# TLeconte/vdlm2dec

Measured on AMD Instinct MI355X. Metric: IQ MS/s demodulated (8 ch, 2 MS/s cs16) + CRC-pass frame parity vs ref, higher is better.
Workload: dtype f32

## Files before the change

### vdlm2dec_amd/csrc/vdl2gpu.hip

```cpp
#include "vdl2gpu_kernels.h"
#include "vdl2gpu_blocks.h"

#include <algorithm>
#include <cmath>
#include <cstdio>
#include <cstdlib>
#include <chrono>
#include <cstring>
#include <mutex>
#include <new>
#include <string>
#include <type_traits>
#include <vector>

extern "C" void sincosf(float, float *, float *);

#define HIPCHK(h, expr)                                                                         \
	do {                                                                                    \
		hipError_t e__ = (expr);                                                        \
		if (e__ != hipSuccess) {                                                        \
			(h)->err = std::string(#expr) + ": " + hipGetErrorString(e__);          \
			return VDL2GPU_EHIP;                                                    \
		}                                                                               \
	} while (0)
// ... 982 lines not shown
	HIPCHK(h, hipStreamSynchronize(h->stream));
	return VDL2GPU_OK;
}

extern "C" int vdl2gpu_create(const vdl2gpu_config_t *cfg, vdl2gpu_t **out)
{
	if (!cfg || !out || cfg->struct_size != sizeof(vdl2gpu_config_t))
		return VDL2GPU_EINVAL;
	if (cfg->nbch < 1 || cfg->nbch > VDL2GPU_MAXCH || cfg->nstreams < 1 || !cfg->chan || !cfg->max_push)
		return VDL2GPU_EINVAL;
	if (fmt_bytes(cfg->fmt) == 0 || cfg->sdrinrate < 100000)
		return VDL2GPU_EINVAL;
	const bool offgrid = cfg->sdrinrate % 25000 != 0;
	if (offgrid && (cfg->sdrinrate % 1000 || (cfg->flags & VDL2GPU_F_RTL_QUIRK)))
		return VDL2GPU_EINVAL;
	if ((cfg->flags & VDL2GPU_F_RTL_QUIRK) && cfg->fmt != VDL2GPU_FMT_CU8)
		return VDL2GPU_EINVAL;
	if (cfg->flags & VDL2GPU_F_EXACT_FO) {
		if (cfg->flags & VDL2GPU_F_RTL_QUIRK)
			return VDL2GPU_EINVAL;
		for (size_t i = 0; i < (size_t)cfg->nstreams * cfg->nbch; ++i)
			if (2ll * std::llabs((long long)cfg->chan[i].Fo) >= (long long)cfg->sdrinrate)
				return VDL2GPU_EINVAL;
	}
#ifndef VDL2GPU_TESTHOOKS
	if (cfg->flags & VDL2GPU_F_TEST_NOREGION)
		return VDL2GPU_EINVAL;
#endif
	const unsigned sdrclk = cfg->sdrclk ? cfg->sdrclk : cfg->sdrinrate / 4000;
	if (sdrclk <= 21 || sdrclk > 1000000)
		return VDL2GPU_EINVAL;
	const unsigned lo_len = (unsigned)vdl2gpu_lo_len(cfg->sdrinrate);
	if (offgrid) {
		if ((4ull * sdrclk) % lo_len || k1_win_bytes((sdrclk + 20) / 21) > VDL2_K1_LDS_MAX)
			return VDL2GPU_EINVAL;
	} else if (k1_smem_bytes(lo_len, (sdrclk + 20) / 21) > VDL2_K1_LDS_MAX)
		return VDL2GPU_EINVAL;
	const long long cap = plane_frames(cfg->max_push, sdrclk);
	if (cap == 0 || (unsigned long long)cap * VDL2_CS * sizeof(float2) >= VDL2_PLANES_MAX)
		return VDL2GPU_EINVAL;
	vdl2gpu_t *h = new(std::nothrow) vdl2gpu;
	if (!h)
		return VDL2GPU_ENOMEM;
	h->cfg = *cfg;
	h->S = cfg->nstreams;
	h->C = cfg->nbch;
	h->L = (int)lo_len;
	h->sdrclk = (int)sdrclk;
	h->maxwin = (h->sdrclk + 20) / 21;
	h->k1_glo = offgrid && k1_smem_bytes((uint64_t)h->L, (uint64_t)h->maxwin) > VDL2_K1_LDS_MAX;
	h->sample_bytes = fmt_bytes(cfg->fmt);
	h->rec_cap = cfg->max_bursts ? cfg->max_bursts : 65536u;
	h->chans.assign(cfg->chan, cfg->chan + (size_t)cfg->nstreams * cfg->nbch);
	h->cfg.chan = h->chans.data();
	const int rc = create_impl(h);
	if (rc != VDL2GPU_OK) {
		std::string e = h->err;
		if (getenv("VDL2GPU_VERBOSE"))
			fprintf(stderr, "vdl2gpu_create: %s\n", e.c_str());
		vdl2gpu_destroy(h);
		*out = nullptr;
		return rc;
	}
	*out = h;
	return VDL2GPU_OK;
}

static int get_events(vdl2gpu_t *h, PushTiming &pt)
{
	if (!h->free_ev.empty()) {
		pt = h->free_ev.back();
		h->free_ev.pop_back();
		return VDL2GPU_OK;
	}
	for (auto &e : pt.e)
		NEW_EVENT(h, e, true);
	return VDL2GPU_OK;
}

static int harvest_timing(vdl2gpu_t *h)
{
	for (auto &pt : h->pending) {
		float d[NEV - 1] = {0};
		if (h->stage_dump && pt.staged && h->ev_origin) {
			static const int order[] = {0, 1, 10, 4, 2, 13, 23, 14, 12, 15, 16, 18, 5, 20, 21, 22, 6, 7};
			fprintf(stderr, "vdl2gpu stage dump push %llu:", (unsigned long long)pt.index);
			for (int k : order) {
				float t = -1.0f;
				if (hipEventElapsedTime(&t, h->ev_origin, pt.e[k]) != hipSuccess) {
					(void)hipGetLastError();
					t = -1.0f;
				}
				fprintf(stderr, " e%d=%.1f", k, t * 1e3f);
			}
			fprintf(stderr, "\n");
		}
		for (int i = 0; i + 1 < NEV; ++i) {
			if (!pt.staged)
				break;
			if (i == 3)
				HIPCHK(h, hipEventElapsedTime(&d[i], pt.e[13], pt.e[14]));
			else
				HIPCHK(h, hipEventElapsedTime(&d[i], i == 1 ? pt.e[10] : (i == 4 ? pt.e[12] : pt.e[i]), i == 1 ? pt.e[4] : pt.e[i + 1]));
		}
		if (pt.fast && pt.staged) {
			float a = 0, b = 0, c = 0;
			HIPCHK(h, hipEventElapsedTime(&a, pt.e[0], pt.e[11]));
			HIPCHK(h, hipEventElapsedTime(&b, pt.e[8], pt.e[9]));
			HIPCHK(h, hipEventElapsedTime(&c, pt.e[9], pt.e[1]));
			d[0] = a + b + c;
		}
		if (pt.staged) {
			h->st_k1 += d[0];
			h->st_scan += d[1] + d[4];
			h->st_cluster += d[2];
			h->st_resolve += d[3] + d[5];
			h->st_demod += d[1] + d[2] + d[3] + d[4] + d[5];
			h->st_other += d[6];
			h->st_pushes++;
		}
		if (pt.fast && pt.staged) {
			float f = 0;
			HIPCHK(h, hipEventElapsedTime(&f, pt.e[8], pt.e[9]));
			h->tm.channelise_fast_ms += f;
			h->tm.fast_pushes++;
		}
		h->tm.pushes++;
		h->tm.samples += pt.samples;
		h->free_ev.push_back(pt);
	}
	h->pending.clear();
	return VDL2GPU_OK;
}

static int harvest_ring(vdl2gpu_t *h, int ring, bool blocking);
static int enqueue_back(vdl2gpu_t *h);
static void spill_slab(vdl2gpu_t *h, int slab);

enum { SCAN_PROBE, SCAN_REGION, SCAN_VERIFY };
struct ScanDrain { int slot = -1, mode = 0, skip = 0, pch = 0, nwg = 0; };
static void scan_drain(K2Params &q, const ScanDrain &d)
{
	q.drain_slot = d.slot;
	q.drain_mode = d.mode;
	q.drain_skip = d.skip;
	q.drain_pch = d.pch;
	q.drain_nwg = d.nwg;
}
static ScanDrain launch_scan(int which, const K2Params &k2, dim3 grid, hipStream_t st, int slot, int mode, int skip, unsigned tiles_per_wg)
{
	K2Params q = k2;
	const unsigned item_priv = k2.item_priv;
	grid.x = std::min<unsigned>(grid.x, VDL2_MAXWG);
	if (which != SCAN_VERIFY)
		grid.x = std::max(1u, std::min<unsigned>(grid.x, item_priv / 256u));
	unsigned want = (tiles_per_wg * (which == SCAN_REGION ? 400u : 42u * (K2A_TS / 1024u)) + 128u + 255u) / 256u * 256u;
	q.surv_common_cap = 0;
#ifdef VDL2GPU_TESTHOOKS
	const bool test_items = !g_test_item_verify || which == SCAN_VERIFY;
	if (test_items && g_test_item_grid > 0) {
		grid.x = std::min<unsigned>(grid.x, (unsigned)g_test_item_grid);
		want = 256u;
	}
	if (test_items && g_test_item_common > 0)
		q.surv_common_cap = g_test_item_common;
#endif
	q.surv_nwg = (int)grid.x;
	q.surv_pch = (int)std::max(256u, std::min(want, item_priv / grid.x / 256u * 256u));
	q.surv_slot = slot;
	q.surv_mode = mode;
	q.surv_skip = skip;
	q.drain_slot = -1;
	switch (which) {
	case SCAN_PROBE: hipLaunchKernelGGL(k2a_probe, grid, dim3(K2A_THREADS), 0, st, q); break;
	case SCAN_REGION: hipLaunchKernelGGL(k2a_region, grid, dim3(K2A_THREADS), 0, st, q); break;
	default: hipLaunchKernelGGL(k2a_verify, grid, dim3(K2A_THREADS), 0, st, q); break;
	}
	ScanDrain d;
	d.slot = slot;
	d.mode = mode;
	d.skip = skip;
	d.pch = q.surv_pch;
	d.nwg = q.surv_nwg;
	return d;
}

template <class F> static void with_fmt(int fmt, F &&f)
{
	switch (fmt) {
	case VDL2GPU_FMT_CU8: f(std::integral_constant<int, VDL2GPU_FMT_CU8>{}); break;
	case VDL2GPU_FMT_CS16: f(std::integral_constant<int, VDL2GPU_FMT_CS16>{}); break;
	case VDL2GPU_FMT_CF32: f(std::integral_constant<int, VDL2GPU_FMT_CF32>{}); break;
	case VDL2GPU_FMT_CS8: f(std::integral_constant<int, VDL2GPU_FMT_CS8>{}); break;
	case VDL2GPU_FMT_S16R: f(std::integral_constant<int, VDL2GPU_FMT_S16R>{}); break;
	default: f(std::integral_constant<int, VDL2GPU_FMT_F32R>{}); break;
	}
}

static int push_impl(vdl2gpu_t *h, const void *iq, size_t nsamples, size_t stream_stride_bytes, int memkind, bool wait_copy);

static int push_checked(vdl2gpu_t *h, const void *iq, size_t nsamples, size_t stream_stride_bytes, int memkind, bool wait_copy)
{
	if (h && h->failed) {
		h->err = "an earlier HIP error left the handle unusable: " + h->err;
		return VDL2GPU_EHIP;
	}
	int rc = VDL2GPU_OK;
	const size_t lim = h ? h->split_samples : 0;
	auto passes = [&](const void *q, size_t n) -> int { return push_impl(h, q, n, stream_stride_bytes, memkind, wait_copy); };
	if (!h || !iq || lim == 0 || nsamples <= lim)
		rc = passes(iq, nsamples);
	else {
		if (nsamples > h->cfg.max_push)
			return VDL2GPU_EINVAL;
		const size_t parts = (nsamples + lim - 1) / lim;
		const size_t unit = h->split_unit;
		const size_t part = ((nsamples + parts - 1) / parts + unit - 1) / unit * unit;
		for (size_t off = 0; off < nsamples && rc == VDL2GPU_OK; off += part)
			rc = passes((const char *)iq + off * h->sample_bytes, std::min(part, nsamples - off));
	}
	if (rc == VDL2GPU_EHIP)
		h->failed = true;
	return rc;
}

extern "C" int vdl2gpu_push(vdl2gpu_t *h, const void *iq, size_t nsamples, size_t stream_stride_bytes, int memkind)
{
	if (!h)
		return VDL2GPU_EINVAL;
	HLOCK(h);
	return push_checked(h, iq, nsamples, stream_stride_bytes, memkind, true);
}

extern "C" int vdl2gpu_ring_init(vdl2gpu_t *h, size_t slot_samples, int nslots)
{
	if (!h || slot_samples == 0 || slot_samples > h->cfg.max_push || nslots < 2 || nslots > 64)
		return VDL2GPU_EINVAL;
	HLOCK(h);
	if (h->ring_host) {
		h->err = "vdl2gpu_ring_init: the ring exists already";
		return VDL2GPU_EINVAL;
	}
	HIPCHK(h, hipSetDevice(h->cfg.device));
	h->ring_slot_samples = slot_samples;
	h->ring_slot_bytes = slot_samples * h->sample_bytes * (size_t)h->S;
	HOST_ALLOC(h, h->ring_host, h->ring_slot_bytes * (size_t)nslots, hipHostMallocDefault);
	h->ring_nslots = nslots;
	h->ring_copied.resize((size_t)nslots);
	h->ring_inflight.assign((size_t)nslots, 0);
	for (int i = 0; i < nslots; ++i)
		NEW_EVENT(h, h->ring_copied[(size_t)i]);
	return VDL2GPU_OK;
}

extern "C" void *vdl2gpu_ring_acquire(vdl2gpu_t *h, size_t *stream_stride_bytes)
{
	if (!h)
		return nullptr;
	HLOCK(h);
	if (!h->ring_host || h->ring_acquired)
		return nullptr;
	const size_t slot = (size_t)(h->ring_next % (unsigned long long)h->ring_nslots);
	if (h->ring_inflight[slot]) {
		if (hipSetDevice(h->cfg.device) != hipSuccess || hipEventSynchronize(h->ring_copied[slot]) != hipSuccess) {
			h->err = "vdl2gpu_ring_acquire: waiting for the slot failed";
			return nullptr;
		}
		h->ring_inflight[slot] = 0;
	}
	if (stream_stride_bytes)
		*stream_stride_bytes = h->ring_slot_samples * h->sample_bytes;
	h->ring_acquired = true;
	return (char *)h->ring_host + slot * h->ring_slot_bytes;
}

extern "C" int vdl2gpu_ring_commit(vdl2gpu_t *h, size_t nsamples)
{
	if (!h)
		return VDL2GPU_EINVAL;
	HLOCK(h);
	if (!h->ring_host || !h->ring_acquired || nsamples > h->ring_slot_samples)
		return VDL2GPU_EINVAL;
	const size_t slot = (size_t)(h->ring_next % (unsigned long long)h->ring_nslots);
	h->ring_acquired = false;
	h->ring_next++;
	if (nsamples == 0)
		return VDL2GPU_OK;
	const int rc = push_checked(h, (char *)h->ring_host + slot * h->ring_slot_bytes, nsamples,
				    h->ring_slot_samples * h->sample_bytes, VDL2GPU_MEM_HOST, false);
	if (h->in_stream) {
		if (hipEventRecord(h->ring_copied[slot], h->in_stream) == hipSuccess)
			h->ring_inflight[slot] = 1;
		else if (rc == VDL2GPU_OK) {
			h->err = "hipEventRecord(ring_copied)";
			h->failed = true;
			return VDL2GPU_EHIP;
		}
	}
	return rc;
}


static inline void (*k2d_kernel(const vdl2gpu_t *h))(K2Params)
{
	return h->col_on[COL_SOFT] ? (h->col_on[COL_LEVEL] ? k2d_payload_lev_soft : k2d_payload_soft) : (h->col_on[COL_LEVEL] ? k2d_payload_lev : k2d_payload);
}

static int enqueue_back(vdl2gpu_t *h)
{
	if (!h->back.valid)
		return VDL2GPU_OK;
	h->back.valid = false;
	const K2Params &k2 = h->back.k2;
	const int64_t J = h->back.J;
	const int par = h->back.par, ring = h->back.ring;
	const bool staged = h->back.staged, serial = h->back.serial;
	const unsigned tiles = h->back.tiles;
	const int GS = h->S;
	PushTiming &pt = h->pending[h->back.pt_index];
	const dim3 gch((unsigned)h->C, (unsigned)GS);
	hipStream_t rs = h->stream;
	if (h->back.two_streams)
		HIPCHK(h, hipStreamWaitEvent(rs, h->set[par].f_done, 0));
	if (staged)
		HIPCHK(h, hipEventRecord(pt.e[2], rs));
	if (!serial)
		hipLaunchKernelGGL(k2b_clusters, dim3((unsigned)(h->n_cu * 4 * K2B_GRIDW), (unsigned)((GS * VDL2_CS + 63) / 64)), dim3(K2B_NT), 0, rs, k2);
	HIPCHK(h, hipGetLastError());
	if (staged)
		HIPCHK(h, hipEventRecord(pt.e[3], rs));
	if (staged)
		HIPCHK(h, hipEventRecord(pt.e[13], rs));
	const dim3 vgrid0((tiles / 2 + 1 + K2A_VRUN - 1) / K2A_VRUN, (unsigned)h->C, (unsigned)GS);
	ScanDrain vdrain;
	if (h->k2f_rec)
		HIPCHK(h, hipStreamWaitEvent(rs, h->k2f_done, 0));
	if (staged && h->stage_dump)
		HIPCHK(h, hipEventRecord(pt.e[23], rs));
	hipLaunchKernelGGL(k2c_resolve, gch, dim3(K2_NT), 0, rs, k2);
	HIPCHK(h, hipGetLastError());
	if (staged)
		HIPCHK(h, hipEventRecord(pt.e[14], rs));
	const bool spec = !h->full_scan && !serial && h->S * VDL2_CS <= 512;
	h->ring[ring].spec = spec;
	if (spec)
		HIPCHK(h, hipEventRecord(h->k2c_done, rs));
	hipStream_t ps = h->copy_stream;
	if (spec) {
		HIPCHK(h, hipStreamWaitEvent(ps, h->k2c_done, 0));
		hipLaunchKernelGGL(k2d_kernel(h), dim3((unsigned)h->k2d_grid, (unsigned)(VDL2_CS * GS)), dim3(K2D_NT), 0, ps, k2);
		HIPCHK(h, hipEventRecord(h->pay_done, ps));
	}
	if (staged)
		HIPCHK(h, hipEventRecord(pt.e[12], h->stream));
	if (!serial)
		vdrain = launch_scan(SCAN_VERIFY, k2, vgrid0, h->stream, VDL2_SURV_VERIFY, 1, 0, K2A_VRUN);
	HIPCHK(h, hipGetLastError());
	if (staged && h->stage_dump)
		HIPCHK(h, hipEventRecord(pt.e[15], h->stream));
	hipStream_t ts = (spec && h->back.two_streams && !h->knob.no_tail) ? h->pay_stream : h->stream;
	if (ts != h->stream) {
		HIPCHK(h, hipEventRecord(h->verify_done, h->stream));
		HIPCHK(h, hipStreamWaitEvent(ts, h->verify_done, 0));
	}
	if (h->tail_prev && h->tail_prev != ts && h->set[(par + VDL2_NSET - 1) % VDL2_NSET].k2_rec)
		HIPCHK(h, hipStreamWaitEvent(ts, h->set[(par + VDL2_NSET - 1) % VDL2_NSET].k2_done, 0));
	h->tail_prev = ts;
	if (staged && h->stage_dump)
		HIPCHK(h, hipEventRecord(pt.e[16], ts));
	if (!h->full_scan && !serial) {
		K2Params k2r = k2;
		if (spec && h->repair_rounds >= 2 && ts != ps)
			HIPCHK(h, hipStreamWaitEvent(ts, h->pay_done, 0));
		const dim3 vgrid((tiles / 2 + 1 + K2A_VRUN - 1) / K2A_VRUN, (unsigned)h->C, (unsigned)GS);
		for (int rr = 1; rr <= h->repair_rounds; ++rr) {
			k2r.round = rr;
			k2r.full_round = (rr == h->repair_rounds && h->repair_rounds >= 2) ? 1 : 0;
			k2r.mini_round = k2r.full_round ? 0 : 1;
			if (k2r.full_round) {
				scan_drain(k2r, vdrain);
				hipLaunchKernelGGL(k2r_regions, gch, dim3(K2R_NT), 0, ts, k2r);
				scan_drain(k2r, ScanDrain());
				const unsigned want = tiles;
				unsigned per = (unsigned)h->n_cu;
				per = per > want ? want : per;
				const ScanDrain pdrain = launch_scan(SCAN_PROBE, k2r, dim3(per, (unsigned)h->C, (unsigned)GS), ts, VDL2_SURV_FULL, 0, 0, 4 * ((want + per - 1) / per));
				scan_drain(k2r, pdrain);
				hipLaunchKernelGGL(k2s_sort, gch, dim3(K2S_NT), 0, ts, k2r);
				scan_drain(k2r, ScanDrain());
				hipLaunchKernelGGL(k2b_clusters, dim3((unsigned)(h->n_cu * 4 * K2B_GRIDW), (unsigned)((GS * VDL2_CS + 63) / 64)), dim3(K2B_NT), 0, ts, k2r);
				hipLaunchKernelGGL(k2c_resolve, gch, dim3(K2_NT), 0, ts, k2r);
				vdrain = ScanDrain();
			} else if (rr == 1) {
				scan_drain(k2r, vdrain);
				hipLaunchKernelGGL(k2p_patch, gch, dim3(K2P_NT), 0, ts, k2r);
				if (staged && h->stage_dump)
					HIPCHK(h, hipEventRecord(pt.e[18], ts));
				scan_drain(k2r, ScanDrain());
				{
					const unsigned nv = std::min<unsigned>(vgrid.x, (unsigned)h->knob.verify2_wg);
					const dim3 vnarrow(nv, vgrid.y, vgrid.z);
					vdrain = launch_scan(SCAN_VERIFY, k2r, vnarrow, ts, VDL2_SURV_VERIFY + rr, 1, 0, K2A_VRUN * ((vgrid.x + nv - 1) / nv));
				}
			} else {
				scan_drain(k2r, vdrain);
				hipLaunchKernelGGL(k2s_merge, gch, dim3(K2M_NT), 0, ts, k2r);
				scan_drain(k2r, ScanDrain());
				hipLaunchKernelGGL(k2c_resolve, gch, dim3(K2_NT), 0, ts, k2r);
				vdrain = launch_scan(SCAN_VERIFY, k2r, vgrid, ts, VDL2_SURV_VERIFY + rr, 1, 0, K2A_VRUN);
			}
		}
		HIPCHK(h, hipGetLastError());
	}
	if (staged)
		HIPCHK(h, hipEventRecord(pt.e[5], ts));
	{
		K2Params k2f = k2;
		scan_drain(k2f, vdrain);
		hipLaunchKernelGGL(k2f_commit, gch, dim3(K2_NT), 0, ts, k2f);
	}

	HIPCHK(h, hipEventRecord(h->k2f_done, ts));
	h->k2f_rec = true;
	if (staged && h->stage_dump)
		HIPCHK(h, hipEventRecord(pt.e[20], ts));
	if (h->ring[ring].spec) {
		if (ts != ps)
			HIPCHK(h, hipStreamWaitEvent(ts, h->pay_done, 0));
		if (!h->full_scan && !serial) {
			K2Params k2p = k2;
			k2p.sel_mode = 1;
			hipLaunchKernelGGL(k2d_kernel(h), dim3((unsigned)h->k2d_grid, (unsigned)(VDL2_CS * GS)), dim3(K2D_NT), 0, ts, k2p);
		}
	} else {
		K2Params k2p = k2;
		k2p.sel_mode = 2;
		hipLaunchKernelGGL(k2d_kernel(h), dim3((unsigned)h->k2d_grid, (unsigned)(VDL2_CS * GS)), dim3(K2D_NT), 0, ts, k2p);
	}
	HIPCHK(h, hipGetLastError());
	if (staged && h->stage_dump)
		HIPCHK(h, hipEventRecord(pt.e[21], ts));
	if (h->frames_on) {
		K4Params k4{};
		k4.recs = h->ring[ring].d_recs;
		k4.nrecs_dev = h->d_outc + 2 * ring;
		k4.rec_cap = h->rec_cap;
		k4.frames = h->ring[ring].d_frames;
		k4.nframes = h->d_fcnt + 4 * ring;
		k4.frame_cap = h->frame_cap;
		k4.compact = 1;
		k4.tabs = h->d_k4tab;
		k4.fmask = h->ring[ring].spec ? h->set[par].k2.fmask : nullptr;
		k4.dbg = h->knob.debug_counters ? h->d_dbg : nullptr;
		k4.soft = h->ring[ring].soft();
		hipLaunchKernelGGL(k4_frames, dim3((unsigned)h->n_cu * 16), dim3(K4_NT), 0, ts, k4);
		HIPCHK(h, hipGetLastError());
	}
	if (staged)
		HIPCHK(h, hipEventRecord(pt.e[6], ts));
	{
		K3Params k3{};
		k3.src = nullptr;
		k3.dst = nullptr;
		k3.cap = h->cap;
		k3.nbch = h->C;
		k3.J = J;
		k3.ss = h->d_ss;
		k3.cs = h->d_cs;
		k3.outc = h->d_outc;
		k3.fmask = h->set[par].k2.fmask;
		k3.fcnt = h->frames_on ? h->d_fcnt + 4 * ring : nullptr;
		k3.host_cnt = h->d_pin_cnt + 32 * ring;
		k3.ring = ring;
		k3.ctl = h->set[par].k2.ctl;
		k3.nstreams = h->S;
		{
			KExportParams ke{};
			ke.recs = h->ring[ring].d_recs;
			ke.count = h->d_outc + 2 * ring;
			ke.dst = h->slab[h->back.slab].d_recs;
			ke.cap = std::min(h->slab_cap, h->rec_cap);
			ke.lev = h->ring[ring].levels();
			ke.ldst = h->slab[h->back.slab].d_levels();
			ke.soft = h->ring[ring].soft();
			ke.sdst = h->slab[h->back.slab].d_soft();
			hipLaunchKernelGGL(k_export_records, dim3((unsigned)h->n_cu), dim3(256), 0, ts, ke);
			HIPCHK(h, hipGetLastError());
			if (staged && h->stage_dump)
				HIPCHK(h, hipEventRecord(pt.e[22], ts));
		}
		hipLaunchKernelGGL(k3_rebase, dim3((unsigned)GS), dim3(64), 0, ts, k3);
		HIPCHK(h, hipGetLastError());
	}
	if (staged)
		HIPCHK(h, hipEventRecord(pt.e[7], ts));
	HIPCHK(h, hipEventRecord(h->set[par].k2_done, ts));
	h->set[par].k2_rec = true;
	h->ring[ring].ev ^= 1;
	HIPCHK(h, hipEventRecord(h->ring[ring].done(), ts));
	return VDL2GPU_OK;
}


struct Input {
	const void *src;
	size_t stride;
	bool staged;
};

static int stage_input(vdl2gpu_t *h, const void *iq, size_t nsamples, size_t stream_stride_bytes, int memkind, bool wait_copy, int stg, Input &in)
{
	in = Input{ iq, stream_stride_bytes, false };
	if (memkind == VDL2GPU_MEM_DEVICE)
		return VDL2GPU_OK;
	if (memkind != VDL2GPU_MEM_HOST)
		return VDL2GPU_EINVAL;
	const size_t per = nsamples * h->sample_bytes;
	const size_t need = per * (size_t)h->S;
	if (!h->in_stream) {
		NEW_STREAM(h, h->in_stream);
		for (int i = 0; i < 2; ++i)
			NEW_EVENT(h, h->raw_copied[i]);
	}
	if (need > h->raw_bytes[stg]) {
		HIPCHK(h, hipStreamSynchronize(h->fstream));
		HIPCHK(h, hipStreamSynchronize(h->stream));
		HIPCHK(h, hipStreamSynchronize(h->pay_stream));
		HIPCHK(h, hipStreamSynchronize(h->in_stream));
		dev_release(h, h->d_raw[stg]);
		h->d_raw[stg] = nullptr;
		h->raw_bytes[stg] = 0;
		DEV_ALLOC(h, h->d_raw[stg], need);
		h->raw_bytes[stg] = need;
	}
	if (h->k1_rec[stg])
		HIPCHK(h, hipStreamWaitEvent(h->in_stream, h->k1_done[stg], 0));
	for (int s = 0; s < h->S; ++s)
		HIPCHK(h, hipMemcpyAsync((char *)h->d_raw[stg] + (size_t)s * per,
					 (const char *)iq + (size_t)s * stream_stride_bytes, per,
					 hipMemcpyHostToDevice, h->in_stream));
	HIPCHK(h, hipEventRecord(h->raw_copied[stg], h->in_stream));
	if (wait_copy)
		HIPCHK(h, hipEventSynchronize(h->raw_copied[stg]));
	in = Input{ h->d_raw[stg], per, true };
	return VDL2GPU_OK;
}

static inline long long wend_abs(long long j, int sdrclk, int c0)
{
	return ((j + 1) * (long long)sdrclk - c0 + 20) / 21 - 1;
}

enum { K1_GENERAL, K1_PP, K1_FAST };
struct K1Choice {
	int kind;
	bool whole;
	long long per_lo;
	long long sbase0;
	int d;
};
static K1Choice choose_k1(const vdl2gpu_t *h, int c0, int64_t J, size_t nsamples, const void *src, size_t stride)
{
// ... 1284 lines not shown
```

### vdlm2dec_amd/csrc/vdl2gpu_scan.h

```cpp
#ifndef VDL2GPU_SCAN_H
#define VDL2GPU_SCAN_H

#ifndef K2A_THREADS
#define K2A_THREADS 256
#endif
#ifndef K2A_TS
#define K2A_TS 1024
#endif
#ifndef K2A_PREFETCH
#define K2A_PREFETCH 0
#endif
#ifndef K2A_FLUSH_ATTR
#define K2A_FLUSH_ATTR
#endif
#ifndef K2A_WPE
#define K2A_WPE 6
#endif
#define K2A_POFF 132
#define K2A_XOFF (K2A_POFF + 16)
#define K2A_XMAX (2 * K2A_TS + K2A_XOFF)
#define K2X_WL 40
#define K2X_NT 256
#define K2X_CV 64
#define VDL2_ITEM_CAP 196608
// ... 877 lines not shown
			const int b = tid * RUN + k;
			if (b < WGS_NBK) {
				const unsigned cnt = ws.cur[b];
				ws.start[b] = run;
				ws.cur[b] = run;
				run += cnt;
			}
		}
		if (tid == NT - 1)
			ws.start[WGS_NBK] = run;
	}
	__syncthreads();
	for (int i = tid; i < n; i += NT) {
		const unsigned long long v = keys[i];
		unsigned b = (unsigned)(v >> tshift) >> bsh;
		b = b < WGS_NBK ? b : WGS_NBK - 1;
		ws.tmp[atomicAdd(&ws.cur[b], 1u)] = v;
	}
	__syncthreads();
	for (int i = tid; i < n; i += NT) {
		const unsigned long long v = ws.tmp[i];
		unsigned b = (unsigned)(v >> tshift) >> bsh;
		b = b < WGS_NBK ? b : WGS_NBK - 1;
		const int lo = (int)ws.start[b], hi = (int)ws.start[b + 1];
		int rank = 0;
		for (int j = lo; j < hi; ++j)
			rank += (ws.tmp[j] < v) ? 1 : 0;
		keys[lo + rank] = v;
	}
	__syncthreads();
}

static_assert(sizeof(K2xWork) <= sizeof(unsigned long long) * VDL2_CAND_CAP, "K2xWork overlays WgSortShared.tmp");
#define K2R_NT 1024
__global__ __launch_bounds__(K2R_NT)
void k2r_regions(K2Params p)
{
	__shared__ unsigned long long key64[VDL2_CAND_CAP];
	__shared__ WgSortShared ws;
	__shared__ int key[VDL2_CAND_CAP];
	const int tid = threadIdx.x;
	const int c = blockIdx.x, s = (int)blockIdx.y;
	const int sc = s * VDL2_CS + c;
	k2x_drain<K2R_NT>(*reinterpret_cast<K2xWork *>(ws.tmp), p, sc);
	if (p.force_serial || p.full_scan)
		return;
	if (p.round > 0 && p.fail[sc] >= VDL2_VERIFIED)
		return;
	if (p.round > 0 && !p.full_round)
		return;
	if (p.full_round) {
		if (tid == 0) {
			p.ctl[CTL_CAND0 + sc] = 0;
			p.ctl[CTL_CAND0 + p.nstreams * VDL2_CS + sc] = 0;
			p.ctl[CTL_NCLUST0 + sc] = 0;
			p.ctl[CTL_NREG0 + sc] = 0;
			p.ctl[CTL_NSEED0 + sc] = 0;
		}
		return;
	}
	int ncand = (int)p.ctl[CTL_NSEED0 + sc];
	ncand = ncand > VDL2_CAND_CAP ? VDL2_CAND_CAP : ncand;
	const int *seeds = p.seeds + (size_t)sc * VDL2_CAND_CAP;
	for (int i = tid; i < ncand; i += K2R_NT)
		key64[i] = ((unsigned long long)(unsigned)seeds[i] << 16) | (unsigned)i;
	__syncthreads();
	wg_sort_u64<K2R_NT>(key64, ws, ncand, 16, (unsigned)(VDL2_CARRY_FRAMES + p.J));
	for (int i = tid; i < ncand; i += K2R_NT)
		key[i] = (int)(key64[i] >> 16);
	__syncthreads();
	{
		__shared__ int s_nreg;
		const int lo_lim = (int)(p.scan_lo - p.dec_base);
		const int hi_lim = (int)(VDL2_CARRY_FRAMES + p.J);
		int2 *regs = p.regs + (size_t)sc * VDL2_REG_CAP;
		if (tid == 0)
			s_nreg = 0;
		__syncthreads();
		for (int i = tid; i < ncand; i += K2R_NT) {
			if (i > 0 && key[i] - key[i - 1] <= VDL2_REG_GAP)
				continue;
			int j = i;
			while (j + 1 < ncand && key[j + 1] - key[j] <= VDL2_REG_GAP)
				++j;
			int lo = key[i] - VDL2_REG_PAD, hi = key[j] + VDL2_REG_PAD + 1;
			lo = lo < lo_lim ? lo_lim : lo;
			hi = hi > hi_lim ? hi_lim : hi;
			if (hi <= lo)
				continue;
			const int nchunk = (hi - lo + K2A_TS - 1) / K2A_TS;
			const int base = atomicAdd(&s_nreg, nchunk);
			for (int k = 0; k < nchunk; ++k)
				if (base + k < VDL2_REG_CAP) {
					const int q = lo + k * K2A_TS;
					regs[base + k] = make_int2(q, (hi - q < K2A_TS) ? hi - q : K2A_TS);
				}
		}
		__syncthreads();
		if (tid == 0) {
			const int n = s_nreg;
			p.ctl[CTL_NREG0 + sc] = (unsigned)(n > VDL2_REG_CAP ? VDL2_REG_CAP : n);
			p.ctl[CTL_NSEED0 + sc] = 0;
		}
	}
}

#ifndef K2A_WPE_REGION
#define K2A_WPE_REGION 5
#endif
__global__ __launch_bounds__(K2A_THREADS) __attribute__((amdgpu_waves_per_eu(K2A_WPE_REGION, 8)))
void k2a_region(K2Params p)
{
	__shared__ K2aShared sh;
	const int c = blockIdx.y, s = (int)blockIdx.z;
	const int sc = s * VDL2_CS + c;
	if (p.force_serial || p.full_scan)
		return;
#ifdef VDL2GPU_TESTHOOKS
	if (p.test_noregion && p.round == 0)
		return;
#endif
	const unsigned nreg = p.ctl[CTL_NREG0 + sc];
	if (blockIdx.x >= nreg)
		return;
	const long long dec_base = p.dec_base;
	const int2 *regs = p.regs + (size_t)sc * VDL2_REG_CAP;
	const int skip_r = p.probe_r, skip_par = p.probe_par;
	if (threadIdx.x < 16)
		sh.prof[threadIdx.x] = 0;
	k2a_tables(sh);
	K2aPre<1> pre;
	pre.loaded = false;
	pre.tiles = 0;
	const bool prof = p.dbg && threadIdx.x == 0 && (blockIdx.x & 7) == 0;
	const long long t0 = prof ? clock64() : 0;
	for (unsigned k = blockIdx.x; k < nreg; k += gridDim.x) {
		const int2 rg = regs[k];
		const int2 rn = (k + gridDim.x < nreg) ? regs[k + gridDim.x] : make_int2(0, 0);
		k2a_tile<1>(sh, p, sc, dec_base, dec_base + rg.x, rg.y, 0xfu, 0, 0, 0, nullptr, pre, dec_base + rn.x, rn.y, skip_r, skip_par);
		if (prof)
			sh.prof[15] += (unsigned long long)rg.y;
	}
	const long long t1 = prof ? clock64() : 0;
	if (prof)
		sh.prof[12] += (unsigned long long)(t1 - t0);
	k2a_tail(sh, sc);
	if (p.dbg && threadIdx.x < 16 && sh.prof[threadIdx.x])
		atomicAdd(p.dbg + 48 + threadIdx.x, sh.prof[threadIdx.x]);
}

#ifndef K2A_VRUN
#define K2A_VRUN 4
#endif
#define K2A_VITEMS 64
__global__ __launch_bounds__(K2A_THREADS) __attribute__((amdgpu_waves_per_eu(K2A_WPE, 8)))
void k2a_verify(K2Params p)
{
	__shared__ K2aShared sh;
	__shared__ int s_list[64], s_nl, s_ni;
	__shared__ int4 s_item[K2A_VITEMS];
	const int tid = threadIdx.x;
	const int c = blockIdx.y, s = (int)blockIdx.z;
	const int sc = s * VDL2_CS + c;
	if (p.force_serial || p.full_scan || p.full_round)
		return;
	if (p.round > 0 && !p.redo[sc])
		return;
	const long long dec_base = p.dec_base;
	const int t_end = (int)(VDL2_CARRY_FRAMES + p.J);
	const int nseg = (int)p.ctl[CTL_NSEG0 + sc];
	const Seg *segs = p.segs + (size_t)sc * VDL2_SEG_CAP;
	if (nseg == 0 || (int)(p.cs[sc].pos - dec_base) + (int)blockIdx.x * K2A_VRUN * 2 * K2A_TS >= t_end)
		return;
	k2a_tables(sh);
	K2aPre<2> pre;
	pre.loaded = false;
	pre.tiles = 0;
	for (int run = (int)blockIdx.x;; run += (int)gridDim.x) {
		const int r_lo = (int)(p.cs[sc].pos - dec_base) + run * K2A_VRUN * 2 * K2A_TS;
		if (r_lo >= t_end)
			break;
		const int r_hi = r_lo + K2A_VRUN * 2 * K2A_TS < t_end ? r_lo + K2A_VRUN * 2 * K2A_TS : t_end;
		__syncthreads();
		if (tid == 0)
			s_nl = 0;
		__syncthreads();
		for (int k = tid; k < nseg && k < VDL2_SEG_CAP; k += K2A_THREADS) {
			const Seg g = segs[k];
			if (g.lo < r_hi && g.hi > r_lo && g.hi > g.lo) {
				const int q = atomicAdd(&s_nl, 1);
				if (q < 64)
					s_list[q] = k;
			}
		}
		__syncthreads();
		const int nl = s_nl;
		if (nl == 0)
			continue;
		if (tid == 0) {
			int ni = 0;
			for (int q = 0; q < nl && q < 64; ++q) {
				const Seg g = segs[s_list[q]];
				for (int t_lo = r_lo; t_lo < r_hi; t_lo += 2 * K2A_TS) {
					const int t_hi = t_lo + 2 * K2A_TS < r_hi ? t_lo + 2 * K2A_TS : r_hi;
					int lo = g.lo > t_lo ? g.lo : t_lo;
					const int hi = g.hi < t_hi ? g.hi : t_hi;
					lo += (lo ^ g.lo) & 1;
					if (lo >= hi)
						continue;
					if (ni < K2A_VITEMS)
						s_item[ni] = make_int4(lo, hi, g.r, 0);
					++ni;
				}
			}
			s_ni = ni;
		}
		__syncthreads();
		const int ni = s_ni;
		if (nl > 64 || ni > K2A_VITEMS) {
			if (tid == 0)
				atomicMin(p.fail + sc, 0);
			break;
		}
		for (int q = 0; q < ni; ++q) {
			const int4 it = s_item[q];
			const int4 nx = (q + 1 < ni) ? s_item[q + 1] : make_int4(0, 0, 0, 0);
			k2a_tile<2>(sh, p, sc, dec_base, dec_base + it.x, (it.y - it.x + 1) / 2, 1u << it.z, 1, dec_base + it.x, dec_base + it.y,
				    p.fail + sc, pre, dec_base + nx.x, (nx.y - nx.x + 1) / 2);
		}
	}
	k2a_tail(sh, sc);
}

#endif
```

Baseline: 175,600.

## Rebalance verify scan over segment tiles with a resident grid and prefix-sum work split

The verify kernel stops assigning fixed time windows to workgroups. It now counts the tiles covered by live segments, builds a block-wide DPP prefix sum, and hands each workgroup an equal contiguous share of those tiles. By default the grid is sized to a resident count, about six workgroups per CU split across channels, and the survivor-buffer share is derived from that size. This targets load imbalance and empty windows, and drops the serial thread-0 item construction. The cost is an extra pass over the segment list and additional block-wide scans and barriers. The old overflow fallback (atomicMin on fail) is removed, and the segment count is clamped instead.

```diff
diff --git a/vdlm2dec_amd/csrc/vdl2gpu.hip b/vdlm2dec_amd/csrc/vdl2gpu.hip
--- a/vdlm2dec_amd/csrc/vdl2gpu.hip
+++ b/vdlm2dec_amd/csrc/vdl2gpu.hip
@@ -1158,8 +1158,7 @@
 	K2Params q = k2;
 	const unsigned item_priv = k2.item_priv;
 	grid.x = std::min<unsigned>(grid.x, VDL2_MAXWG);
-	if (which != SCAN_VERIFY)
-		grid.x = std::max(1u, std::min<unsigned>(grid.x, item_priv / 256u));
+	grid.x = std::max(1u, std::min<unsigned>(grid.x, item_priv / 256u));
 	unsigned want = (tiles_per_wg * (which == SCAN_REGION ? 400u : 42u * (K2A_TS / 1024u)) + 128u + 255u) / 256u * 256u;
 	q.surv_common_cap = 0;
 #ifdef VDL2GPU_TESTHOOKS
@@ -1189,6 +1188,12 @@
 	d.pch = q.surv_pch;
 	d.nwg = q.surv_nwg;
 	return d;
+}
+
+static unsigned verify_share(unsigned pieces, unsigned nwg)
+{
+	nwg = std::max(1u, std::min<unsigned>(nwg, VDL2_MAXWG));
+	return (pieces + nwg - 1) / nwg + 1;
 }
 
 template <class F> static void with_fmt(int fmt, F &&f)
@@ -1337,7 +1342,13 @@
 		HIPCHK(h, hipEventRecord(pt.e[3], rs));
 	if (staged)
 		HIPCHK(h, hipEventRecord(pt.e[13], rs));
-	const dim3 vgrid0((tiles / 2 + 1 + K2A_VRUN - 1) / K2A_VRUN, (unsigned)h->C, (unsigned)GS);
+	const unsigned vpieces = tiles / 2 + 1;
+#if K2A_VGRID_RESIDENT
+	const unsigned vwg0 = std::min(vpieces, std::max(1u, (unsigned)h->n_cu * 6u / (unsigned)(h->C * GS)));
+#else
+	const unsigned vwg0 = (vpieces + K2A_VRUN - 1) / K2A_VRUN;
+#endif
+	const dim3 vgrid0(vwg0, (unsigned)h->C, (unsigned)GS);
 	ScanDrain vdrain;
 	if (h->k2f_rec)
 		HIPCHK(h, hipStreamWaitEvent(rs, h->k2f_done, 0));
@@ -1360,7 +1371,7 @@
 	if (staged)
 		HIPCHK(h, hipEventRecord(pt.e[12], h->stream));
 	if (!serial)
-		vdrain = launch_scan(SCAN_VERIFY, k2, vgrid0, h->stream, VDL2_SURV_VERIFY, 1, 0, K2A_VRUN);
+		vdrain = launch_scan(SCAN_VERIFY, k2, vgrid0, h->stream, VDL2_SURV_VERIFY, 1, 0, verify_share(vpieces, vgrid0.x));
 	HIPCHK(h, hipGetLastError());
 	if (staged && h->stage_dump)
 		HIPCHK(h, hipEventRecord(pt.e[15], h->stream));
@@ -1378,7 +1389,7 @@
 		K2Params k2r = k2;
 		if (spec && h->repair_rounds >= 2 && ts != ps)
 			HIPCHK(h, hipStreamWaitEvent(ts, h->pay_done, 0));
-		const dim3 vgrid((tiles / 2 + 1 + K2A_VRUN - 1) / K2A_VRUN, (unsigned)h->C, (unsigned)GS);
+		const dim3 vgrid(vgrid0);
 		for (int rr = 1; rr <= h->repair_rounds; ++rr) {
 			k2r.round = rr;
 			k2r.full_round = (rr == h->repair_rounds && h->repair_rounds >= 2) ? 1 : 0;
@@ -1404,16 +1415,16 @@
 					HIPCHK(h, hipEventRecord(pt.e[18], ts));
 				scan_drain(k2r, ScanDrain());
 				{
-					const unsigned nv = std::min<unsigned>(vgrid.x, (unsigned)h->knob.verify2_wg);
+					const unsigned nv = std::min<unsigned>(vpieces, (unsigned)h->knob.verify2_wg);
 					const dim3 vnarrow(nv, vgrid.y, vgrid.z);
-					vdrain = launch_scan(SCAN_VERIFY, k2r, vnarrow, ts, VDL2_SURV_VERIFY + rr, 1, 0, K2A_VRUN * ((vgrid.x + nv - 1) / nv));
+					vdrain = launch_scan(SCAN_VERIFY, k2r, vnarrow, ts, VDL2_SURV_VERIFY + rr, 1, 0, verify_share(vpieces, nv));
 				}
 			} else {
 				scan_drain(k2r, vdrain);
 				hipLaunchKernelGGL(k2s_merge, gch, dim3(K2M_NT), 0, ts, k2r);
 				scan_drain(k2r, ScanDrain());
 				hipLaunchKernelGGL(k2c_resolve, gch, dim3(K2_NT), 0, ts, k2r);
-				vdrain = launch_scan(SCAN_VERIFY, k2r, vgrid, ts, VDL2_SURV_VERIFY + rr, 1, 0, K2A_VRUN);
+				vdrain = launch_scan(SCAN_VERIFY, k2r, vgrid, ts, VDL2_SURV_VERIFY + rr, 1, 0, verify_share(vpieces, vgrid.x));
 			}
 		}
 		HIPCHK(h, hipGetLastError());
diff --git a/vdlm2dec_amd/csrc/vdl2gpu_scan.h b/vdlm2dec_amd/csrc/vdl2gpu_scan.h
--- a/vdlm2dec_amd/csrc/vdl2gpu_scan.h
+++ b/vdlm2dec_amd/csrc/vdl2gpu_scan.h
@@ -1053,12 +1053,83 @@
 #ifndef K2A_VRUN
 #define K2A_VRUN 4
 #endif
+#ifndef K2A_VGRID_RESIDENT
+#define K2A_VGRID_RESIDENT 1
+#endif
 #define K2A_VITEMS 64
+
+__device__ __forceinline__ int k2a_vseg(const Seg *segs, int k, int nseg, int p_lo, int t_end, int &lo, int &hi, int &r)
+{
+	lo = hi = r = 0;
+	if (k >= nseg)
+		return 0;
+	const Seg g = segs[k];
+	lo = g.lo > p_lo ? g.lo : p_lo;
+	lo += (lo ^ g.lo) & 1;
+	hi = g.hi < t_end ? g.hi : t_end;
+	r = g.r & 3;
+	if (g.hi <= g.lo || hi <= lo) {
+		hi = lo;
+		return 0;
+	}
+	return ((hi - lo + 1) / 2 + K2A_TS - 1) / K2A_TS;
+}
+
+__device__ __forceinline__ int k2a_vscan(int v, int *s_w, int &total)
+{
+	int incl = v;
+	incl += __builtin_amdgcn_update_dpp(0, incl, 0x111, 0xf, 0xf, false);
+	incl += __builtin_amdgcn_update_dpp(0, incl, 0x112, 0xf, 0xf, false);
+	incl += __builtin_amdgcn_update_dpp(0, incl, 0x114, 0xf, 0xf, false);
+	incl += __builtin_amdgcn_update_dpp(0, incl, 0x118, 0xf, 0xf, false);
+	incl += __builtin_amdgcn_update_dpp(0, incl, 0x142, 0xa, 0xf, false);
+	incl += __builtin_amdgcn_update_dpp(0, incl, 0x143, 0xc, 0xf, false);
+	__syncthreads();
+	if ((threadIdx.x & 63) == 63)
+		s_w[threadIdx.x >> 6] = incl;
+	__syncthreads();
+	int base = 0, tot = 0;
+#pragma unroll
+	for (int w = 0; w < K2A_THREADS / 64; ++w) {
+		const int t = s_w[w];
+		base += (w < (int)(threadIdx.x >> 6)) ? t : 0;
+		tot += t;
+	}
+	total = tot;
+	return base + incl - v;
+}
+
+template <bool FIRST> __device__ __forceinline__ void k2a_vitems(const Seg *segs, int nseg, int p_lo, int t_end, int a, int b, int lo0, int hi0, int r0,
+								  int n0, int *s_w, int4 *s_item)
+{
+	int carry = 0;
+	for (int k0 = 0; k0 < nseg && carry < b; k0 += K2A_THREADS) {
+		int lo, hi, r, n;
+		if (FIRST && k0 == 0) {
+			lo = lo0;
+			hi = hi0;
+			r = r0;
+			n = n0;
+		} else
+			n = k2a_vseg(segs, k0 + (int)threadIdx.x, nseg, p_lo, t_end, lo, hi, r);
+		int tot;
+		const int e = carry + k2a_vscan(n, s_w, tot);
+		carry += tot;
+		int j = a > e ? a - e : 0;
+		const int j1 = (b - e < n) ? b - e : n;
+		for (; j < j1; ++j) {
+			const int l = lo + j * 2 * K2A_TS;
+			s_item[e + j - a] = make_int4(l, (hi - l > 2 * K2A_TS) ? l + 2 * K2A_TS : hi, r, 0);
+		}
+	}
+	__syncthreads();
+}
+
 __global__ __launch_bounds__(K2A_THREADS) __attribute__((amdgpu_waves_per_eu(K2A_WPE, 8)))
 void k2a_verify(K2Params p)
 {
 	__shared__ K2aShared sh;
-	__shared__ int s_list[64], s_nl, s_ni;
+	__shared__ int s_w[K2A_THREADS / 64];
 	__shared__ int4 s_item[K2A_VITEMS];
 	const int tid = threadIdx.x;
 	const int c = blockIdx.y, s = (int)blockIdx.z;
@@ -1069,66 +1140,57 @@
 		return;
 	const long long dec_base = p.dec_base;
 	const int t_end = (int)(VDL2_CARRY_FRAMES + p.J);
-	const int nseg = (int)p.ctl[CTL_NSEG0 + sc];
+	int nseg = (int)p.ctl[CTL_NSEG0 + sc];
+	nseg = nseg < 0 || nseg > VDL2_SEG_CAP ? VDL2_SEG_CAP : nseg;
 	const Seg *segs = p.segs + (size_t)sc * VDL2_SEG_CAP;
-	if (nseg == 0 || (int)(p.cs[sc].pos - dec_base) + (int)blockIdx.x * K2A_VRUN * 2 * K2A_TS >= t_end)
-		return;
+	if (nseg == 0)
+		return;
+	const int p_lo = (int)(p.cs[sc].pos - dec_base);
+	int lo0, hi0, r0;
+	const int n0 = k2a_vseg(segs, tid, nseg, p_lo, t_end, lo0, hi0, r0);
+	int T;
+	{
+		int mine = n0;
+		for (int k = K2A_THREADS + tid; k < nseg; k += K2A_THREADS) {
+			int lo, hi, r;
+			mine += k2a_vseg(segs, k, nseg, p_lo, t_end, lo, hi, r);
+		}
+		k2a_vscan(mine, s_w, T);
+	}
+	const int G = (int)gridDim.x;
+	const int q = (T + G - 1) / G;
+	int ch = (int)blockIdx.x;
+	int a = ch * q;
+	if (a >= T)
+		return;
+	int c_end = a + q < T ? a + q : T;
 	k2a_tables(sh);
 	K2aPre<2> pre;
 	pre.loaded = false;
 	pre.tiles = 0;
-	for (int run = (int)blockIdx.x;; run += (int)gridDim.x) {
-		const int r_lo = (int)(p.cs[sc].pos - dec_base) + run * K2A_VRUN * 2 * K2A_TS;
-		if (r_lo >= t_end)
-			break;
-		const int r_hi = r_lo + K2A_VRUN * 2 * K2A_TS < t_end ? r_lo + K2A_VRUN * 2 * K2A_TS : t_end;
-		__syncthreads();
-		if (tid == 0)
-			s_nl = 0;
-		__syncthreads();
-		for (int k = tid; k < nseg && k < VDL2_SEG_CAP; k += K2A_THREADS) {
-			const Seg g = segs[k];
-			if (g.lo < r_hi && g.hi > r_lo && g.hi > g.lo) {
-				const int q = atomicAdd(&s_nl, 1);
-				if (q < 64)
-					s_list[q] = k;
-			}
-		}
-		__syncthreads();
-		const int nl = s_nl;
-		if (nl == 0)
-			continue;
-		if (tid == 0) {
-			int ni = 0;
-			for (int q = 0; q < nl && q < 64; ++q) {
-				const Seg g = segs[s_list[q]];
-				for (int t_lo = r_lo; t_lo < r_hi; t_lo += 2 * K2A_TS) {
-					const int t_hi = t_lo + 2 * K2A_TS < r_hi ? t_lo + 2 * K2A_TS : r_hi;
-					int lo = g.lo > t_lo ? g.lo : t_lo;
-					const int hi = g.hi < t_hi ? g.hi : t_hi;
-					lo += (lo ^ g.lo) & 1;
-					if (lo >= hi)
-						continue;
-					if (ni < K2A_VITEMS)
-						s_item[ni] = make_int4(lo, hi, g.r, 0);
-					++ni;
-				}
-			}
-			s_ni = ni;
-		}
-		__syncthreads();
-		const int ni = s_ni;
-		if (nl > 64 || ni > K2A_VITEMS) {
-			if (tid == 0)
-				atomicMin(p.fail + sc, 0);
-			break;
-		}
-		for (int q = 0; q < ni; ++q) {
-			const int4 it = s_item[q];
-			const int4 nx = (q + 1 < ni) ? s_item[q + 1] : make_int4(0, 0, 0, 0);
+	int b = a + K2A_VITEMS < c_end ? a + K2A_VITEMS : c_end;
+	k2a_vitems<true>(segs, nseg, p_lo, t_end, a, b, lo0, hi0, r0, n0, s_w, s_item);
+	for (;;) {
+		const int ni = b - a;
+		if (p.dbg && tid < ni)
+			atomicAdd(p.dbg + 30, (unsigned long long)((s_item[tid].y - s_item[tid].x + 1) / 2));
+		for (int i = 0; i < ni; ++i) {
+			const int4 it = s_item[i];
+			const int4 nx = (i + 1 < ni) ? s_item[i + 1] : make_int4(0, 0, 0, 0);
 			k2a_tile<2>(sh, p, sc, dec_base, dec_base + it.x, (it.y - it.x + 1) / 2, 1u << it.z, 1, dec_base + it.x, dec_base + it.y,
 				    p.fail + sc, pre, dec_base + nx.x, (nx.y - nx.x + 1) / 2);
 		}
+		a = b;
+		if (a >= c_end) {
+			ch += G;
+			a = ch * q;
+			if (a >= T)
+				break;
+			c_end = a + q < T ? a + q : T;
+		}
+		b = a + K2A_VITEMS < c_end ? a + K2A_VITEMS : c_end;
+		__syncthreads();
+		k2a_vitems<false>(segs, nseg, p_lo, t_end, a, b, 0, 0, 0, 0, s_w, s_item);
 	}
 	k2a_tail(sh, sc);
 }
```

New measurement: 184,100, median of 6. 4.8% higher.
